# craftsangjae/instance-segmentation-road-project

Measured on AMD Instinct MI355X. Metric: images/sec at 1024x1024 (MaskLab inference hot path, full forward), higher is better.
Workload: dtype f32; 1 GPU; resnext50_full_b8_1024; per_gpu_batch=8, global_batch=8, height=1024, width=1024, parallelism=dp1, hipgraph=False, inputs=resident in HBM, weights=random init (cls logits x8 so NMS / mask head run at full load)

## Files before the change

### include/masklab_hip.h

```cpp
#ifndef MASKLAB_HIP_H
#define MASKLAB_HIP_H

#include <stdint.h>

#ifdef __cplusplus
extern "C" {
#endif

#define ML_OK 0
#define ML_E_BADARG (-1)
#define ML_E_LAUNCH (-2)
#define ML_E_NOGPU  (-3)

enum { ML_ACT_NONE = 0, ML_ACT_RELU = 1, ML_ACT_RELU6 = 2, ML_ACT_SIGMOID = 3 };
enum { ML_MATH_F32 = 0, ML_MATH_F16 = 1, ML_MATH_F16S = 2, ML_MATH_F32X3 = 3 };

#define ML_ABI_VERSION 7
int ml_version(void);
const char *ml_last_error(void);
int ml_device_check(void);

typedef struct ml_conv2d_desc {
    const float *in;
    const float *wgt;
// ... 25 lines not shown
} ml_conv2d_desc;

int ml_conv2d_f32(const ml_conv2d_desc *d, void *stream);

#define ML_CONV_MAX_PROBLEMS 12
int64_t ml_conv2d_workspace_bytes(void);
int ml_conv2d_multi_f32(const ml_conv2d_desc *descs, int32_t n, void *workspace, int64_t workspace_bytes,
                        void *stream);
int ml_conv2d_ntile(int32_t cout, int32_t tile);
int ml_conv2d_launch_ntile(const ml_conv2d_desc *descs, int32_t n, int32_t has_workspace);
int ml_conv2d_launch_mtile(const ml_conv2d_desc *descs, int32_t n, int32_t has_workspace);
int ml_conv2d_uses_pipe(const ml_conv2d_desc *d);
int ml_conv2d_launch_splits(const ml_conv2d_desc *descs, int32_t n, int64_t workspace_bytes, int32_t *splits);
int ml_conv2d_wino_eligible(const ml_conv2d_desc *d);
int ml_conv2d_wino_narrow(const ml_conv2d_desc *d);
int64_t ml_conv2d_gn_min_launch_tiles(void);

int ml_gconv3x3_f32(const float *in, const float *wgt, const float *bias, float *out,
                    int32_t B, int32_t H, int32_t W, int32_t C, int32_t c, int32_t Ho, int32_t Wo,
                    int32_t stride, int32_t pad_t, int32_t pad_l, int32_t act, void *stream);

int ml_gconv3x3_f16(const void *in, const float *wgt, const float *bias, void *out,
                    int32_t B, int32_t H, int32_t W, int32_t C, int32_t c, int32_t Ho, int32_t Wo,
                    int32_t stride, int32_t pad_t, int32_t pad_l, int32_t act, void *stream);

int ml_gconv3x3_launch_plan(int32_t B, int32_t H, int32_t W, int32_t C, int32_t c, int32_t stride, int32_t Ho, int32_t Wo,
                            int32_t is_half, int32_t plan[6]);

int ml_maxpool3x3s2_f16(const void *in, void *out, int32_t B, int32_t H, int32_t W, int32_t C,
                        int32_t Ho, int32_t Wo, int32_t pad_t, int32_t pad_l, void *stream);
// ... 397 lines not shown
```

### instance-segmentation-road-project_amd/csrc/conv_mfma.hip

```cpp
#include "gfx_mem.h"

namespace {

constexpr int LDS_LD = 32;
constexpr int LDS_LD_H = 40;

constexpr int MAXP = ML_CONV_MAX_PROBLEMS;

struct FastDiv { unsigned mul; int shift; };

static FastDiv make_fastdiv(unsigned d) {
    FastDiv f;
    if (d <= 1) { f.mul = 0; f.shift = -1; return f; }
    int s = 0;
    while ((1ull << s) < d) ++s;
    const unsigned long long num = 1ull << (31 + s);
    f.mul = (unsigned)((num + d - 1) / d);
    f.shift = s - 1;
    return f;
}

__device__ __forceinline__ int fast_div(int n, const FastDiv f) {
    return f.shift < 0 ? n : (int)(__umulhi((unsigned)n, f.mul) >> f.shift);
}
// ... 992 lines not shown
                       "vector epilogue (out / bias 16-byte aligned, out_cstride and out_coff multiples of 4)");
        p.start[i] = (int)start;
        start += (MB + 7) / 8 * 8 * (d.n_pad / p.BN) * splits;
        ML_REQUIRE(start < (1ll << 31), "conv2d: grid too large");
    }
    p.start[p.n] = (int)start;
    return ML_OK;
}

}

int ml_conv1x1_pipe_try(const ml_conv2d_desc &d, hipStream_t s, int *eligible);
int ml_conv1x1_pipe_eligible(const ml_conv2d_desc &d);
int ml_conv1x1_h256_try(const ml_conv2d_desc &d, hipStream_t s, int *took);
int ml_conv1x1_h256_eligible(const ml_conv2d_desc &d);
int ml_conv2d_wino_launch(const ml_conv2d_desc *descs, int n, hipStream_t s);

static bool h256_preferred(const ml_conv2d_desc &d) {
    return d.tile == 5 || (d.tile == 0 && (d.span >= 512 || (d.span >= 256 && d.cout >= 512)));
}

extern "C" int ml_conv2d_ntile(int32_t cout, int32_t tile) {
    const int t = pick_tile(cout, tile);
    return t == 1 ? 128 : (t == 2 ? 64 : 32);
}

extern "C" int64_t ml_conv2d_workspace_bytes(void) { return 512ll << 20; }

static int split_by_image_groups(const ml_conv2d_desc *descs, int n, ConvPlan &p) {
    p.n = 0;
    for (int i = 0; i < n; ++i) {
// ... 128 lines not shown
    }
    ML_REQUIRE(p.kernel < N_GENERIC_KERNELS, "conv2d: no kernel instantiation for math %d, %d x %d tiles", math, p.BM, p.BN);
    return check ? plan_splits(p, ws_bytes) : ML_OK;
}

extern "C" int ml_conv2d_multi_f32(const ml_conv2d_desc *descs, int32_t n, void *workspace, int64_t workspace_bytes,
                                   void *stream) {
    ML_REQUIRE(descs != nullptr && n >= 1 && n <= MAXP, "conv2d: need 1..%d problems", MAXP);
    for (int i = 0; i < n; ++i) {
        ML_REQUIRE(descs[i].in && descs[i].wgt && descs[i].out, "conv2d: null tensor pointer");
        ML_REQUIRE(ml_aligned16(descs[i].in) && ml_aligned16(descs[i].wgt), "conv2d: in/wgt must be 16-byte aligned");
    }
    ConvPlan p;
    if (int rc = plan_launch(descs, n, workspace ? workspace_bytes : 0, p)) return rc;
    hipStream_t s = reinterpret_cast<hipStream_t>(stream);
    if (p.family == CONV_WINO) return ml_conv2d_wino_launch(descs, n, s);
    if (p.family == CONV_H256 || p.family == CONV_PIPE) {
        int took = 0;
        if (int rc = (p.family == CONV_H256 ? ml_conv1x1_h256_try : ml_conv1x1_pipe_try)(descs[0], s, &took)) return rc;
        ML_REQUIRE(took, "conv2d: the persistent 1x1 kernel did not take a problem it was planned for");
        return ML_OK;
    }
    if (workspace) ML_REQUIRE((((uintptr_t)workspace) & 255) == 0, "conv2d: workspace must be 256-byte aligned");
    return kGenericKernels[p.kernel].launch(p, workspace, s);
}


extern "C" int ml_conv2d_uses_pipe(const ml_conv2d_desc *d) {
    ConvPlan p;
    return plan_launch(d, 1, 0, p, false) != ML_OK ? 0 : (p.family == CONV_H256 ? 2 : p.family == CONV_PIPE);
}

extern "C" int ml_conv2d_launch_ntile(const ml_conv2d_desc *descs, int32_t n, int32_t has_workspace) {
    ConvPlan p;
    return plan_launch(descs, n, has_workspace ? ml_conv2d_workspace_bytes() : 0, p, false) == ML_OK && p.family == CONV_GENERIC ? p.BN : 0;
}

extern "C" int ml_conv2d_launch_mtile(const ml_conv2d_desc *descs, int32_t n, int32_t has_workspace) {
    ConvPlan p;
// ... 24 lines not shown
```

### instance-segmentation-road-project_amd/csrc/conv_wino.hip

```cpp
#include "gfx_mem.h"

namespace {

constexpr int WMAXP = ML_CONV_MAX_PROBLEMS;
constexpr int WT = 64;
constexpr int WN = 64;
constexpr int WK = 8;
constexpr int WCHUNK = WK * 32 * 16;
constexpr int WSTEP = 4 * 32 * 16;
constexpr int NSLOT_P = 3;
constexpr int SLOT_P = WT * 16 * 8;
constexpr int NSLOT_W = 4;
constexpr int SLOT_W = 2 * WSTEP;
constexpr int RING_W = NSLOT_P * SLOT_P;
constexpr int LDS_BYTES = (RING_W + NSLOT_W * SLOT_W) * 4;
static_assert(LDS_BYTES == 160 * 1024, "the two rings fill the CU's LDS");
#ifndef WINO_EXP
#define WINO_EXP 0
#endif
constexpr unsigned OOB = 0x80000000u;
constexpr long long SPAN_MAX = 0x7fffff00ll;

struct WProblem {
    ml_conv2d_desc d;
    int TH, TW, T;
    int MB, NB, nchunks;
};

struct WArgs {
    int n;
    int start[WMAXP + 1];
    WProblem p[WMAXP];
};

typedef f32x4 f32x4d __attribute__((aligned(4)));

__device__ __forceinline__ void out_store(float *base, float *ptr, float val) {
#if (WINO_EXP & 8) && defined(__HIP_DEVICE_COMPILE__)
    const __amdgpu_buffer_rsrc_t none = rsrc_bytes(base, 0);
    __builtin_amdgcn_raw_buffer_store_b32(__builtin_bit_cast(unsigned, val), none, (int)((ptr - base) * 4), 0, 0);
#else
// ... 27 lines not shown
            default: v[i * 4 + 3] = t[i * 4 + 1] - t[i * 4 + 3]; break;
        }
    }
}

__global__ void __launch_bounds__(512, 1) conv_wino_kernel(const WArgs args) {
    extern __shared__ __align__(16) float lds[];

    int pi = 0;
    while (pi + 1 < args.n && (int)blockIdx.x >= args.start[pi + 1]) ++pi;
    const WProblem &P = args.p[pi];
    const ml_conv2d_desc &p = P.d;
    const int b = (int)blockIdx.x - args.start[pi];
    const int g = b / (8 * P.NB), rr = b - g * 8 * P.NB;
    const int nt2 = rr >> 3;
    const int mt = g * 8 + (rr & 7);
    if (mt >= P.MB) return;
    if (p.live) {
        const int lv = max(1, *p.live), tpi0 = P.TH * P.TW;
        const int b0 = mt * WT / tpi0, b1 = min(mt * WT + WT, P.T) - 1;
        bool any = false;
        for (int bi = b0; bi <= b1 / tpi0 && !any; ++bi) any = bi % p.live_period < lv;
        if (!any) return;
    }

    const int tid = threadIdx.x, lane = tid & 63;
    const int wave = __builtin_amdgcn_readfirstlane(tid >> 6);
    const int tg = wave & 3, h = wave >> 2;
    const int r = lane & 15, kq = lane >> 4;
    const int tpi = P.TH * P.TW;

    const int gt0 = mt * WT;
    long long base_pix;
    {
        const int bi = gt0 / tpi, rem = gt0 - bi * tpi, ty = rem / P.TW;
        base_pix = ((long long)bi * p.H + max(2 * ty - 1, 0)) * p.W;
    }
    const size_t cstride = (size_t)p.in_cstride;
    const float *pin = p.in + p.in_coff + (size_t)base_pix * cstride;
    int voff_p[4];
    {
        const int rt = (lane >> 1) & 15;
        const int quad = (lane & 1) ^ ((rt >> 2) & 1);
        const int gt = gt0 + (wave >> 1) * 16 + rt;
        int bi = 0, ty = 0, tx = 0;
        if (gt < P.T) {
            bi = gt / tpi;
            const int rem = gt - bi * tpi;
            ty = rem / P.TW;
            tx = rem - ty * P.TW;
        }
#pragma unroll
        for (int i = 0; i < 4; ++i) {
            const int px = 8 * (wave & 1) + 2 * i + (lane >> 5);
            const int y = 2 * ty - 1 + (px >> 2), x = 2 * tx - 1 + (px & 3);
            voff_p[i] = (int)OOB;
            if (gt < P.T && y >= 0 && y < p.H && x >= 0 && x < p.W)
                voff_p[i] = (int)((((long long)bi * p.H + y) * p.W + x - base_pix) * (long long)cstride * 4) + quad * 16;
        }
    }
    const int voff_w = ((wave & 3) * 512 + r * 16 + kq * 4) * 4;
    const float *wsrc = p.wgt + (size_t)(2 * nt2 + (wave >> 2)) * P.nchunks * WCHUNK;
    float *dst_p = lds + (wave >> 1) * 2048 + (wave & 1) * 1024;
    float *dst_w = lds + RING_W + (wave >> 2) * WSTEP + (wave & 3) * 512;
    const int nch = P.nchunks, nsteps = 2 * P.nchunks;
    const bool dead = (2 * nt2 + h) * 32 >= p.cout;

    auto rsrc_p = [&](int j) __attribute__((always_inline)) {
        const bool real = j < nch && !(WINO_EXP & 1);
        return rsrc_bytes(pin + j * 8, real ? (int)OOB : 0);
    };
    auto rsrc_w = [&](int s) __attribute__((always_inline)) {
        const bool real = s < nsteps && !dead && !(WINO_EXP & 2);
        return rsrc_bytes(wsrc + (size_t)s * WSTEP, real ? WSTEP * 4 : 0);
    };

    f32x4 acc[2][16];
#pragma unroll
    for (int t = 0; t < 2; ++t)
#pragma unroll
        for (int q = 0; q < 16; ++q) acc[t][q] = f32x4{0.f, 0.f, 0.f, 0.f};

    const float *pa_lane0 = lds + tg * 2048 + r * 8 + 4 * ((r >> 2) & 1) + kq;
    const float *pa_lane1 = lds + tg * 2048 + r * 8 + 4 * (((r >> 2) & 1) ^ 1) + kq;
    const float *pb_lane = lds + RING_W + h * WSTEP + kq * 512 + r * 4;
    struct Ops {
        float d[16], t[16], v[16];
        f32x4 b[2][4];
    };
    auto read_ops = [&](const float *pa, const float *pb, Ops &o) __attribute__((always_inline)) {
#pragma unroll
        for (int t = 0; t < 2; ++t)
#pragma unroll
            for (int pq = 0; pq < 4; ++pq) o.b[t][pq] = *reinterpret_cast<const f32x4 *>(pb + t * 256 + pq * 64);
#pragma unroll
        for (int px = 0; px < 16; ++px) o.d[px] = pa[px * 128];
// ... 18 lines not shown
#if WINO_EXP != 4
            if (m % 6 == 5 && m / 6 < ndma) {
                __builtin_amdgcn_sched_barrier(0);
                dma(m / 6);
                __builtin_amdgcn_sched_barrier(0);
            }
#endif
            if (m >= 16) {
                bt_d_b_op(2 * (m - 16), nxt.d, nxt.t, nxt.v);
                bt_d_b_op(2 * (m - 16) + 1, nxt.d, nxt.t, nxt.v);
                __builtin_amdgcn_sched_barrier(0);
            }
        }
    };

    {
        const __amdgpu_buffer_rsrc_t rp0 = rsrc_p(0), rp1 = rsrc_p(1), rw0 = rsrc_w(0), rw1 = rsrc_w(1), rw2 = rsrc_w(2);
#pragma unroll
        for (int i = 0; i < 4; ++i) lds_dma16(rp0, (char *)(dst_p + i * 256), voff_p[i], 0);
        lds_dma16(rw0, (char *)dst_w, voff_w, 0);
        lds_dma16(rw0, (char *)(dst_w + 256), voff_w + 1024, 0);
#pragma unroll
        for (int i = 0; i < 4; ++i) lds_dma16(rp1, (char *)(dst_p + SLOT_P + i * 256), voff_p[i], 0);
        lds_dma16(rw1, (char *)(dst_w + SLOT_W), voff_w, 0);
        lds_dma16(rw1, (char *)(dst_w + SLOT_W + 256), voff_w + 1024, 0);
        lds_dma16(rw2, (char *)(dst_w + 2 * SLOT_W), voff_w, 0);
        lds_dma16(rw2, (char *)(dst_w + 2 * SLOT_W + 256), voff_w + 1024, 0);
    }
    wait_vmcnt<8>();
    __builtin_amdgcn_s_barrier();

    if (dead) {
        int ps2 = 2 * SLOT_P;
        for (int j = 0; j < nch; ++j) {
            const int w0 = (2 * j) & 3;
            const int wa = ((w0 ^ 2) + 1) * SLOT_W, wb = w0 * SLOT_W;
            asm volatile("s_waitcnt vmcnt(0) lgkmcnt(0)" ::: "memory");
            __builtin_amdgcn_s_barrier();
            const __amdgpu_buffer_rsrc_t rp = rsrc_p(j + 2), rwa = rsrc_w(2 * j + 3), rwb = rsrc_w(2 * j + 4);
#pragma unroll
            for (int q = 0; q < 8; ++q) {
                if (q < 4) lds_dma16(rp, (char *)(dst_p + ps2 + q * 256), voff_p[q], 0);
                else if (q < 6) lds_dma16(rwa, (char *)(dst_w + wa + (q - 4) * 256), voff_w + (q - 4) * 1024, 0);
                else lds_dma16(rwb, (char *)(dst_w + wb + (q - 6) * 256), voff_w + (q - 6) * 1024, 0);
                __builtin_amdgcn_s_sleep(3);
            }
            ps2 = ps2 == 2 * SLOT_P ? 0 : ps2 + SLOT_P;
        }
        wait_vmcnt<0>();
        return;
    }

    Ops oa, ob;
    read_ops(pa_lane0, pb_lane, oa);
#pragma unroll
    for (int k = 0; k < 32; ++k) bt_d_b_op(k, oa.d, oa.t, oa.v);

    int ps0 = 0, ps1 = SLOT_P, ps2 = 2 * SLOT_P;
    for (int j = 0; j < nch; ++j) {
        const int w0 = (2 * j) & 3;
        const int wa = ((w0 ^ 2) + 1) * SLOT_W, wb = w0 * SLOT_W;
        asm volatile("s_waitcnt vmcnt(0) lgkmcnt(0)" ::: "memory");
        __builtin_amdgcn_s_barrier();
        const __amdgpu_buffer_rsrc_t rp = rsrc_p(j + 2), rwa = rsrc_w(2 * j + 3), rwb = rsrc_w(2 * j + 4);
        auto dma = [&](int q) __attribute__((always_inline)) {
            if (q < 4) lds_dma16(rp, (char *)(dst_p + ps2 + q * 256), voff_p[q], 0);
            else if (q < 6) lds_dma16(rwa, (char *)(dst_w + wa + (q - 4) * 256), voff_w + (q - 4) * 1024, 0);
            else lds_dma16(rwb, (char *)(dst_w + wb + (q - 6) * 256), voff_w + (q - 6) * 1024, 0);
        };
        step(oa, ob, pa_lane1 + ps0, pb_lane + (w0 + 1) * SLOT_W, 5, dma);
        step(ob, oa, pa_lane0 + ps1, pb_lane + (w0 ^ 2) * SLOT_W, 3, [&](int q) __attribute__((always_inline)) { dma(q + 5); });
        const int ps = ps0;
        ps0 = ps1;
        ps1 = ps2;
        ps2 = ps;
    }
    wait_vmcnt<0>();

    const int nt = 2 * nt2 + h;
    const bool gn = p.gn_partials != nullptr && !(WINO_EXP & 16);
    double gs[2] = {0.0, 0.0}, gq[2] = {0.0, 0.0};
    long long f0 = 0;
    if (gn) {
        const int bi = gt0 / tpi, rem = gt0 - bi * tpi, ty = rem / P.TW, tx = rem - ty * P.TW;
        f0 = ((long long)(bi * p.Ho + 2 * ty) * p.Wo + 2 * tx) >> 7;
    }
    const float lo = 0.f, hi = (p.act == ML_ACT_RELU6) ? 6.f : 3.402823466e38f;
    const bool clampv = p.act == ML_ACT_RELU || p.act == ML_ACT_RELU6;
    const int gt = gt0 + tg * 16 + r;
    if (gt < P.T) {
        const int bi = gt / tpi, rem = gt - bi * tpi;
        const int ty = rem / P.TW, tx = rem - ty * P.TW;
        const int oy = 2 * ty, ox = 2 * tx;
        const bool y1 = oy + 1 < p.Ho, x1 = ox + 1 < p.Wo;
        const size_t img = p.out_bstride ? (size_t)bi * (size_t)p.out_bstride : (size_t)bi * p.Ho * p.Wo * p.out_cstride;
        const size_t pix0 = (size_t)oy * p.Wo + ox;
        const long long m_flat0 = (long long)(bi * p.Ho + oy) * p.Wo + ox;
#pragma unroll
        for (int t = 0; t < 2; ++t) {
            const int n = nt * 32 + 16 * t + 4 * kq;
            if (n >= p.cout) continue;
            const bool quad = n + 4 <= p.cout;
            f32x4 u[8];
#pragma unroll
            for (int j = 0; j < 4; ++j) {
                u[j] = acc[t][0 * 4 + j] + acc[t][1 * 4 + j] + acc[t][2 * 4 + j];
                u[4 + j] = acc[t][1 * 4 + j] - acc[t][2 * 4 + j] - acc[t][3 * 4 + j];
            }
            f32x4 bv = {0.f, 0.f, 0.f, 0.f};
            if (p.bias) {
                if (quad) bv = *reinterpret_cast<const f32x4d *>(p.bias + n);
                else
#pragma unroll
                    for (int c = 0; c < 3; ++c)
                        if (n + c < p.cout) bv[c] = p.bias[n + c];
            }
            float *o = p.out + img + p.out_coff + n;
#pragma unroll
            for (int a = 0; a < 2; ++a)
#pragma unroll
                for (int c2 = 0; c2 < 2; ++c2) {
                    if ((a && !y1) || (c2 && !x1)) continue;
                    f32x4 val = (c2 ? u[4 * a + 1] - u[4 * a + 2] - u[4 * a + 3] : u[4 * a + 0] + u[4 * a + 1] + u[4 * a + 2]) + bv;
#pragma unroll
                    for (int c = 0; c < 4; ++c) {
                        if (clampv) val[c] = __builtin_amdgcn_fmed3f(val[c], lo, hi);
                        else if (p.act != ML_ACT_NONE) val[c] = ml_apply_act(val[c], p.act);
                    }
                    float *op = o + (pix0 + (size_t)a * p.Wo + c2) * p.out_cstride;
                    if (quad) out_store(p.out, op, val);
                    else
#pragma unroll
                        for (int c = 0; c < 3; ++c)
                            if (n + c < p.cout) out_store(p.out, op + c, val[c]);
                    if (gn) {
                        const int f = ((m_flat0 + (long long)a * p.Wo + c2) >> 7) != f0;
#pragma unroll
                        for (int c = 0; c < 4; ++c) {
                            gs[f] += (double)val[c];
                            gq[f] += (double)val[c] * (double)val[c];
                        }
                    }
                }
        }
    }
    if (gn) {
        double *lds_gn = reinterpret_cast<double *>(lds);
        __syncthreads();
#pragma unroll
        for (int o = 32; o > 0; o >>= 1) {
#pragma unroll
            for (int f = 0; f < 2; ++f) {
                gs[f] += __shfl_down(gs[f], o, 64);
                gq[f] += __shfl_down(gq[f], o, 64);
            }
        }
        if (lane == 0) {
            lds_gn[wave * 4 + 0] = gs[0]; lds_gn[wave * 4 + 1] = gq[0];
            lds_gn[wave * 4 + 2] = gs[1]; lds_gn[wave * 4 + 3] = gq[1];
        }
        __syncthreads();
        if (tid < 4) {
            const int hh = tid >> 1, ff = tid & 1;
            const int gt1 = gt0 + WT - 1;
            const int bi = gt1 / tpi, rem = gt1 - bi * tpi, ty = rem / P.TW, tx = rem - ty * P.TW;
            const long long f1 = ((long long)(bi * p.Ho + 2 * ty + 1) * p.Wo + 2 * tx + 1) >> 7;
            const long long ft = ff ? f1 : f0;
            const int slot = 2 * nt2 + hh;
            double s = 0.0, q = 0.0;
            for (int w = 0; w < 4; ++w) { s += lds_gn[(hh * 4 + w) * 4 + 2 * ff]; q += lds_gn[(hh * 4 + w) * 4 + 2 * ff + 1]; }
            p.gn_partials[2 * (ft * 4 + slot)] = s;
            p.gn_partials[2 * (ft * 4 + slot) + 1] = q;
        }
    }
}

}

extern "C" int ml_conv2d_wino_eligible(const ml_conv2d_desc *d) {
    if (!d) return 0;
    return d->math == ML_MATH_F32 && d->KH == 3 && d->KW == 3 && d->stride == 1 && d->dil == 1 && d->pad_t == 1 &&
           d->pad_l == 1 && d->Ho == d->H && d->Wo == d->W && d->cpp_shift == 30 && d->group_cin_step == 0 &&
           !d->shuffle2x2 && !d->residual && !d->out_f16 && d->span % 32 == 0 && d->span_pad == d->span &&
           d->cout <= 128 && d->n_pad == 128;
}

extern "C" int ml_conv2d_wino_narrow(const ml_conv2d_desc *d) {
    if (!d || d->live || d->gn_partials) return 0;
    if (d->n_pad != 32 && d->n_pad != 64 && d->n_pad != 96) return 0;
    if (d->cout < 1 || d->cout > d->n_pad || d->cout == 32 || d->cout == 64) return 0;
    ml_conv2d_desc w = *d;
    w.n_pad = 128;
    return ml_conv2d_wino_eligible(&w);
}

int ml_conv2d_wino_gn_ok(const ml_conv2d_desc &d) {
    if (d.Ho % 2 || d.Wo % 2 || d.cout != 128 || d.out_bstride || d.act == ML_ACT_SIGMOID) return 0;
    const long long TH = d.Ho / 2, TW = d.Wo / 2;
    return (64 % TW == 0 || TW % 64 == 0) && (TH * TW) % 64 == 0;
}

int ml_conv2d_wino_launch(const ml_conv2d_desc *descs, int n, hipStream_t s) {
    ML_REQUIRE(n >= 1 && n <= WMAXP, "conv2d (winograd): need 1..%d problems", WMAXP);
    WArgs args;
    args.n = n;
    long long start = 0;
    for (int i = 0; i < n; ++i) {
        const ml_conv2d_desc &d = descs[i];
        ML_REQUIRE(ml_conv2d_wino_eligible(&d),
                   "conv2d: tile = 6 (Winograd F(2x2,3x3)) needs ML_MATH_F32, a 3x3 stride-1 undilated 'same' conv, no "
                   "groups / shuffle / residual / half output, span %% 32 == 0 and n_pad == 128");
        ML_REQUIRE(((d.in_cstride | d.in_coff) & 3) == 0 && ml_aligned16(d.in) && ml_aligned16(d.wgt),
                   "conv2d (winograd): 16-byte aligned input channels and weights");
        if (d.gn_partials)
            ML_REQUIRE(ml_conv2d_wino_gn_ok(d) && !d.live, "conv2d (winograd): gn_partials needs even Ho / Wo, Wo / 2 dividing or a "
                                                "multiple of 64, (Ho / 2) (Wo / 2) %% 64 == 0, cout = 128, dense output");
        WProblem &P = args.p[i];
        P.d = d;
        P.TH = (d.Ho + 1) / 2;
        P.TW = (d.Wo + 1) / 2;
        const long long T = (long long)d.B * P.TH * P.TW;
        ML_REQUIRE(T < (1ll << 30), "conv2d (winograd): too many tiles");
        P.T = (int)T;
        P.MB = (int)((T + WT - 1) / WT);
        P.NB = (d.cout + WN - 1) / WN;
        P.nchunks = d.span_pad / WK;
        const long long span = (2ll * (WT / P.TW + 2) + 2) * d.W * d.in_cstride * 4;
        ML_REQUIRE(span <= SPAN_MAX, "conv2d (winograd): a block's input rows exceed 2 GiB (W x in_cstride too large)");
        args.start[i] = (int)start;
        start += (long long)(P.MB + 7) / 8 * 8 * P.NB;
        ML_REQUIRE(start < (1ll << 31), "conv2d (winograd): grid too large");
    }
    args.start[n] = (int)start;
    long long tiles128 = 0;
    bool any_gn = false;
    for (int i = 0; i < n; ++i) {
        tiles128 += ((long long)descs[i].B * descs[i].Ho * descs[i].Wo + 127) / 128 * (descs[i].n_pad / 128);
        any_gn = any_gn || descs[i].gn_partials != nullptr;
    }
    ML_REQUIRE(!any_gn || tiles128 >= ml_conv2d_gn_min_launch_tiles(),
               "conv2d (winograd): gn_partials needs a launch of ml_conv2d_gn_min_launch_tiles() tiles of 128 x 128");
    static std::atomic<unsigned long long> lds_ok{0};
    if (int rc = ml_ensure_dynamic_lds(reinterpret_cast<const void *>(conv_wino_kernel), LDS_BYTES, lds_ok, "conv2d (winograd)"))
        return rc;
    hipLaunchKernelGGL(conv_wino_kernel, dim3((unsigned)start), dim3(512), LDS_BYTES, s, args);
    ML_CHECK_LAUNCH("conv2d (winograd)");
    return ML_OK;
}
// ... 1 lines not shown
```

### instance-segmentation-road-project_amd/masklab_hip/_lib.py

```python
import ctypes as C
import os

_HERE = os.path.dirname(os.path.abspath(__file__))
LIB_PATH = os.path.join(_HERE, "libmasklab_hip.so")

ABI_VERSION = 7
ACT_NONE, ACT_RELU, ACT_RELU6, ACT_SIGMOID = 0, 1, 2, 3
ACT_BY_NAME = {None: ACT_NONE, "linear": ACT_NONE, "relu": ACT_RELU, "relu6": ACT_RELU6,
               "sigmoid": ACT_SIGMOID}


class ConvDesc(C.Structure):
    _fields_ = [
        ("in_", C.c_void_p), ("wgt", C.c_void_p), ("bias", C.c_void_p),
        ("residual", C.c_void_p), ("out", C.c_void_p),
        ("B", C.c_int32), ("H", C.c_int32), ("W", C.c_int32),
        ("in_cstride", C.c_int32), ("in_coff", C.c_int32),
        ("span", C.c_int32), ("span_pad", C.c_int32), ("cpp_shift", C.c_int32),
        ("Ho", C.c_int32), ("Wo", C.c_int32),
        ("KH", C.c_int32), ("KW", C.c_int32), ("stride", C.c_int32), ("dil", C.c_int32),
        ("pad_t", C.c_int32), ("pad_l", C.c_int32),
        ("cout", C.c_int32), ("n_pad", C.c_int32),
        ("out_cstride", C.c_int32), ("out_coff", C.c_int32),
        ("res_cstride", C.c_int32), ("res_coff", C.c_int32),
# ... 74 lines not shown
DECONV_OUT_MAX_PROBLEMS = 4
_i32, _i64, _f32, _f64, _vp = C.c_int32, C.c_int64, C.c_float, C.c_double, C.c_void_p

SIGNATURES = {
    "ml_version": (C.c_int, []),
    "ml_last_error": (C.c_char_p, []),
    "ml_device_check": (C.c_int, []),
    "ml_conv2d_f32": (C.c_int, [C.POINTER(ConvDesc), _vp]),
    "ml_conv2d_ntile": (C.c_int, [_i32, _i32]),
    "ml_conv2d_uses_pipe": (C.c_int, [C.POINTER(ConvDesc)]),
    "ml_conv2d_launch_ntile": (C.c_int, [C.POINTER(ConvDesc), _i32, _i32]),
    "ml_conv2d_launch_mtile": (C.c_int, [C.POINTER(ConvDesc), _i32, _i32]),
    "ml_conv2d_launch_splits": (C.c_int, [C.POINTER(ConvDesc), _i32, _i64, C.POINTER(C.c_int32)]),
    "ml_conv2d_wino_eligible": (C.c_int, [C.POINTER(ConvDesc)]),
    "ml_conv2d_wino_narrow": (C.c_int, [C.POINTER(ConvDesc)]),
    "ml_conv2d_gn_min_launch_tiles": (_i64, []),
    "ml_conv2d_workspace_bytes": (_i64, []),
    "ml_conv2d_multi_f32": (C.c_int, [C.POINTER(ConvDesc), _i32, _vp, _i64, _vp]),
    "ml_deconv2x2_out1x1_f32": (C.c_int, [C.POINTER(DeconvOutProblem), _i32, _i32, _i32, _i32, _i32, _i32, _i32, _vp]),
    "ml_gconv3x3_f32": (C.c_int, [_vp, _vp, _vp, _vp] + [_i32] * 11 + [_vp]),
    "ml_gconv3x3_f16": (C.c_int, [_vp, _vp, _vp, _vp] + [_i32] * 11 + [_vp]),
    "ml_gconv3x3_launch_plan": (C.c_int, [_i32] * 9 + [C.POINTER(C.c_int32)]),
    "ml_maxpool3x3s2_f16": (C.c_int, [_vp, _vp] + [_i32] * 8 + [_vp]),
    "ml_stem7x7s2_pool_f16": (C.c_int, [_vp, _vp, _vp, _vp] + [_i32] * 5 + [_vp]),
    "ml_stem7x7s2_pool_f32": (C.c_int, [_vp, _vp, _vp, _vp] + [_i32] * 5 + [_vp]),
    "ml_stem7x7s2_pool_x3": (C.c_int, [_vp, _vp, _vp, _vp] + [_i32] * 5 + [_vp]),
    "ml_subsample2_f16": (C.c_int, [_vp, _vp] + [_i32] * 4 + [_vp]),
    "ml_cast_f16_to_f32": (C.c_int, [_vp, _vp, _i64, _vp]),
    "ml_cast_f32_to_f16": (C.c_int, [_vp, _vp, _i64, _vp]),
    "ml_resize_bilinear_ac_f16": (C.c_int, [_vp, _vp, _vp] + [_i32] * 12 + [_vp]),
# ... 147 lines not shown
```

### instance-segmentation-road-project_amd/masklab_hip/ops.py

```python
import ctypes as C
import threading

import numpy as np
import torch

from . import _lib
from .packing import PackedConv, pack_winograd, resolve_padding

import weakref

_ws_cache = {}
_ws_retired = []
_graph_owners = weakref.WeakSet()


def graph_owner_registered(model):
    _graph_owners.add(model)


def graph_owner_released(model):
    _graph_owners.discard(model)
    if not len(_graph_owners):
        _ws_retired.clear()

PROFILE = None
LAUNCH_LOG = None


class _Prof:
    def __init__(self, kernel, flops, nbytes, shape=""):
        self.on = PROFILE is not None
        if self.on:
            self.rec = {"kernel": kernel, "flops": float(flops), "bytes": float(nbytes), "shape": shape,
                        "start": torch.cuda.Event(enable_timing=True), "end": torch.cuda.Event(enable_timing=True)}

    def __enter__(self):
        if self.on:
            self.rec["start"].record()
        return self

    def __exit__(self, *exc):
# ... 217 lines not shown
    if wino:
        flops = sum(_wino_flops(descs[i]) for i in range(n))
    ws = workspace(int(lib.ml_conv2d_workspace_bytes()), x.device, "conv")
    if LAUNCH_LOG is not None:
        sp = (C.c_int32 * n)()
        _lib.check(lib.ml_conv2d_launch_splits(descs, n, ws.numel(), sp), "ml_conv2d_launch_splits")
        LAUNCH_LOG.append((" | ".join(shapes) if multi else label, tuple(int(v) for v in sp)))
    name = None
    if PROFILE is not None:
        name = "conv_wino_f32" if wino else _conv_kernel_name(descs, n, dc.p, x.dtype == torch.float16)
    with _Prof(name, flops, nbytes, label) as prof:
        if prof.on and name == "conv1x1_h256_h":
            d = descs[0]
            M, N, K = d.B * d.Ho * d.Wo, d.cout, d.span
            prof.rec["staged_bytes"] = float(-(-M // 256) * (N // 256) * 2 * 256 * K * 2)
        _lib.check(lib.ml_conv2d_multi_f32(descs, n, _ptr(ws), ws.numel(), _stream()), "ml_conv2d_multi_f32")


def _wino_select(descs, n, problems):
    if CONV_MATH != "f32":
        return False
    lib = _lib.load()
    for i, (x, dc) in enumerate(problems):
        if x.dtype != torch.float32 or dc.p.tile != 0:
            return False
        if not (lib.ml_conv2d_wino_eligible(C.byref(descs[i])) or lib.ml_conv2d_wino_narrow(C.byref(descs[i]))):
            return False
    for i, (x, dc) in enumerate(problems):
        descs[i].tile, descs[i].n_pad = 6, 128
        descs[i].wgt = dc.wgt_wino.data_ptr()
    return True
# ... 2047 lines not shown
```

Measured before the change: 436.2 images/sec.

## Make Winograd conv blocks persistent over multiple M panels with cross-panel prefetch

Restructures the Winograd F(2x2,3x3) kernel so one block can loop over several consecutive M panels. The next panel's input and weight DMA is staged into LDS during the current panel's epilogue, and the bias load moves to buffer loads. This is meant to hide prologue latency and cut block launch overhead. The default panel count from wino_class_panels is 1, so the multi-panel path only runs when WINO_PANELS is set, and the default path still carries the restructured loop and extra barriers.

Result: no change. 436.5 images/sec, median of 2 (+0.0%).

```diff
diff --git a/include/masklab_hip.h b/include/masklab_hip.h
--- a/include/masklab_hip.h
+++ b/include/masklab_hip.h
@@ -63,6 +63,8 @@
 int ml_conv2d_launch_splits(const ml_conv2d_desc *descs, int32_t n, int64_t workspace_bytes, int32_t *splits);
 int ml_conv2d_wino_eligible(const ml_conv2d_desc *d);
 int ml_conv2d_wino_narrow(const ml_conv2d_desc *d);
+int ml_conv2d_wino_launch_plan(const ml_conv2d_desc *descs, int32_t n, int32_t *plan);
+int ml_conv2d_multi_wino_panels_f32(const ml_conv2d_desc *descs, int32_t n, const int32_t *panels, void *stream);
 int64_t ml_conv2d_gn_min_launch_tiles(void);
 
 int ml_gconv3x3_f32(const float *in, const float *wgt, const float *bias, float *out,
diff --git a/instance-segmentation-road-project_amd/csrc/conv_mfma.hip b/instance-segmentation-road-project_amd/csrc/conv_mfma.hip
--- a/instance-segmentation-road-project_amd/csrc/conv_mfma.hip
+++ b/instance-segmentation-road-project_amd/csrc/conv_mfma.hip
@@ -1030,7 +1030,7 @@
 int ml_conv1x1_pipe_eligible(const ml_conv2d_desc &d);
 int ml_conv1x1_h256_try(const ml_conv2d_desc &d, hipStream_t s, int *took);
 int ml_conv1x1_h256_eligible(const ml_conv2d_desc &d);
-int ml_conv2d_wino_launch(const ml_conv2d_desc *descs, int n, hipStream_t s);
+int ml_conv2d_wino_launch(const ml_conv2d_desc *descs, int n, const int32_t *panels, hipStream_t s);
 
 static bool h256_preferred(const ml_conv2d_desc &d) {
     return d.tile == 5 || (d.tile == 0 && (d.span >= 512 || (d.span >= 256 && d.cout >= 512)));
@@ -1189,7 +1189,7 @@
     ConvPlan p;
     if (int rc = plan_launch(descs, n, workspace ? workspace_bytes : 0, p)) return rc;
     hipStream_t s = reinterpret_cast<hipStream_t>(stream);
-    if (p.family == CONV_WINO) return ml_conv2d_wino_launch(descs, n, s);
+    if (p.family == CONV_WINO) return ml_conv2d_wino_launch(descs, n, nullptr, s);
     if (p.family == CONV_H256 || p.family == CONV_PIPE) {
         int took = 0;
         if (int rc = (p.family == CONV_H256 ? ml_conv1x1_h256_try : ml_conv1x1_pipe_try)(descs[0], s, &took)) return rc;
@@ -1198,6 +1198,18 @@
     }
     if (workspace) ML_REQUIRE((((uintptr_t)workspace) & 255) == 0, "conv2d: workspace must be 256-byte aligned");
     return kGenericKernels[p.kernel].launch(p, workspace, s);
+}
+
+extern "C" int ml_conv2d_multi_wino_panels_f32(const ml_conv2d_desc *descs, int32_t n, const int32_t *panels, void *stream) {
+    ML_REQUIRE(descs != nullptr && panels != nullptr && n >= 1 && n <= MAXP, "conv2d: need 1..%d problems", MAXP);
+    for (int i = 0; i < n; ++i) {
+        ML_REQUIRE(descs[i].in && descs[i].wgt && descs[i].out, "conv2d: null tensor pointer");
+        ML_REQUIRE(ml_aligned16(descs[i].in) && ml_aligned16(descs[i].wgt), "conv2d: in/wgt must be 16-byte aligned");
+    }
+    ConvPlan p;
+    if (int rc = plan_launch(descs, n, 0, p)) return rc;
+    ML_REQUIRE(p.family == CONV_WINO, "conv2d: panels per block are a choice of the Winograd kernel (tile = 6) only");
+    return ml_conv2d_wino_launch(descs, n, panels, reinterpret_cast<hipStream_t>(stream));
 }
 
 
diff --git a/instance-segmentation-road-project_amd/csrc/conv_wino.hip b/instance-segmentation-road-project_amd/csrc/conv_wino.hip
--- a/instance-segmentation-road-project_amd/csrc/conv_wino.hip
+++ b/instance-segmentation-road-project_amd/csrc/conv_wino.hip
@@ -25,6 +25,7 @@
     ml_conv2d_desc d;
     int TH, TW, T;
     int MB, NB, nchunks;
+    int kp, GB;
 };
 
 struct WArgs {
@@ -82,32 +83,39 @@
     const int b = (int)blockIdx.x - args.start[pi];
     const int g = b / (8 * P.NB), rr = b - g * 8 * P.NB;
     const int nt2 = rr >> 3;
-    const int mt = g * 8 + (rr & 7);
-    if (mt >= P.MB) return;
-    if (p.live) {
-        const int lv = max(1, *p.live), tpi0 = P.TH * P.TW;
-        const int b0 = mt * WT / tpi0, b1 = min(mt * WT + WT, P.T) - 1;
-        bool any = false;
-        for (int bi = b0; bi <= b1 / tpi0 && !any; ++bi) any = bi % p.live_period < lv;
-        if (!any) return;
-    }
+    const int mt_first = (g * 8 + (rr & 7)) * P.kp;
+    const int mt_end = min(mt_first + P.kp, P.MB);
+    const int tpi = P.TH * P.TW;
+    const int lv = p.live ? max(1, *p.live) : 0;
+    auto next_panel = [&](int mt) __attribute__((always_inline)) {
+        for (; mt < mt_end; ++mt) {
+            if (!p.live) break;
+            const int b0 = mt * WT / tpi, b1 = min(mt * WT + WT, P.T) - 1;
+            bool any = false;
+            for (int bi = b0; bi <= b1 / tpi && !any; ++bi) any = bi % p.live_period < lv;
+            if (any) break;
+        }
+        return mt;
+    };
+    int mt = next_panel(mt_first);
+    if (mt >= mt_end) return;
 
     const int tid = threadIdx.x, lane = tid & 63;
     const int wave = __builtin_amdgcn_readfirstlane(tid >> 6);
     const int tg = wave & 3, h = wave >> 2;
     const int r = lane & 15, kq = lane >> 4;
-    const int tpi = P.TH * P.TW;
-
-    const int gt0 = mt * WT;
-    long long base_pix;
-    {
-        const int bi = gt0 / tpi, rem = gt0 - bi * tpi, ty = rem / P.TW;
-        base_pix = ((long long)bi * p.H + max(2 * ty - 1, 0)) * p.W;
-    }
+
     const size_t cstride = (size_t)p.in_cstride;
-    const float *pin = p.in + p.in_coff + (size_t)base_pix * cstride;
+    const float *pin;
     int voff_p[4];
-    {
+    auto panel_geometry = [&](int mtp) __attribute__((always_inline)) {
+        const int gt0 = mtp * WT;
+        long long base_pix;
+        {
+            const int bi = gt0 / tpi, rem = gt0 - bi * tpi, ty = rem / P.TW;
+            base_pix = ((long long)bi * p.H + max(2 * ty - 1, 0)) * p.W;
+        }
+        pin = p.in + p.in_coff + (size_t)base_pix * cstride;
         const int rt = (lane >> 1) & 15;
         const int quad = (lane & 1) ^ ((rt >> 2) & 1);
         const int gt = gt0 + (wave >> 1) * 16 + rt;
@@ -126,7 +134,8 @@
             if (gt < P.T && y >= 0 && y < p.H && x >= 0 && x < p.W)
                 voff_p[i] = (int)((((long long)bi * p.H + y) * p.W + x - base_pix) * (long long)cstride * 4) + quad * 16;
         }
-    }
+    };
+    panel_geometry(mt);
     const int voff_w = ((wave & 3) * 512 + r * 16 + kq * 4) * 4;
     const float *wsrc = p.wgt + (size_t)(2 * nt2 + (wave >> 2)) * P.nchunks * WCHUNK;
     float *dst_p = lds + (wave >> 1) * 2048 + (wave & 1) * 1024;
@@ -144,10 +153,6 @@
     };
 
     f32x4 acc[2][16];
-#pragma unroll
-    for (int t = 0; t < 2; ++t)
-#pragma unroll
-        for (int q = 0; q < 16; ++q) acc[t][q] = f32x4{0.f, 0.f, 0.f, 0.f};
 
     const float *pa_lane0 = lds + tg * 2048 + r * 8 + 4 * ((r >> 2) & 1) + kq;
     const float *pa_lane1 = lds + tg * 2048 + r * 8 + 4 * (((r >> 2) & 1) ^ 1) + kq;
@@ -196,8 +201,10 @@
         }
     };
 
-    {
-        const __amdgpu_buffer_rsrc_t rp0 = rsrc_p(0), rp1 = rsrc_p(1), rw0 = rsrc_w(0), rw1 = rsrc_w(1), rw2 = rsrc_w(2);
+    auto prologue = [&]() __attribute__((always_inline)) {
+        const bool none = (WINO_EXP & 32) != 0;
+        const __amdgpu_buffer_rsrc_t rp0 = rsrc_p(none ? nch : 0), rp1 = rsrc_p(none ? nch : 1);
+        const __amdgpu_buffer_rsrc_t rw0 = rsrc_w(none ? nsteps : 0), rw1 = rsrc_w(none ? nsteps : 1), rw2 = rsrc_w(none ? nsteps : 2);
 #pragma unroll
         for (int i = 0; i < 4; ++i) lds_dma16(rp0, (char *)(dst_p + i * 256), voff_p[i], 0);
         lds_dma16(rw0, (char *)dst_w, voff_w, 0);
@@ -208,152 +215,192 @@
         lds_dma16(rw1, (char *)(dst_w + SLOT_W + 256), voff_w + 1024, 0);
         lds_dma16(rw2, (char *)(dst_w + 2 * SLOT_W), voff_w, 0);
         lds_dma16(rw2, (char *)(dst_w + 2 * SLOT_W + 256), voff_w + 1024, 0);
-    }
+    };
+    auto stage_next = [&](int nx) __attribute__((always_inline)) {
+        if (nx < mt_end) {
+            asm volatile("s_waitcnt vmcnt(0) lgkmcnt(0)" ::: "memory");
+            __builtin_amdgcn_s_barrier();
+            panel_geometry(nx);
+            prologue();
+        }
+    };
+    auto enter_staged = [&]() __attribute__((always_inline)) {
+        asm volatile("s_waitcnt vmcnt(0) lgkmcnt(0)" ::: "memory");
+        __builtin_amdgcn_s_barrier();
+    };
+    auto clear_acc = [&]() __attribute__((always_inline)) {
+#pragma unroll
+        for (int t = 0; t < 2; ++t)
+#pragma unroll
+            for (int q = 0; q < 16; ++q) {
+                acc[t][q] = f32x4{0.f, 0.f, 0.f, 0.f};
+                asm volatile("" : "+v"(acc[t][q]));
+            }
+    };
+    prologue();
+    clear_acc();
     wait_vmcnt<8>();
     __builtin_amdgcn_s_barrier();
 
     if (dead) {
-        int ps2 = 2 * SLOT_P;
+        for (;;) {
+            int ps2 = 2 * SLOT_P;
+            for (int j = 0; j < nch; ++j) {
+                const int w0 = (2 * j) & 3;
+                const int wa = ((w0 ^ 2) + 1) * SLOT_W, wb = w0 * SLOT_W;
+                asm volatile("s_waitcnt vmcnt(0) lgkmcnt(0)" ::: "memory");
+                __builtin_amdgcn_s_barrier();
+                const __amdgpu_buffer_rsrc_t rp = rsrc_p(j + 2), rwa = rsrc_w(2 * j + 3), rwb = rsrc_w(2 * j + 4);
+#pragma unroll
+                for (int q = 0; q < 8; ++q) {
+                    if (q < 4) lds_dma16(rp, (char *)(dst_p + ps2 + q * 256), voff_p[q], 0);
+                    else if (q < 6) lds_dma16(rwa, (char *)(dst_w + wa + (q - 4) * 256), voff_w + (q - 4) * 1024, 0);
+                    else lds_dma16(rwb, (char *)(dst_w + wb + (q - 6) * 256), voff_w + (q - 6) * 1024, 0);
+                    __builtin_amdgcn_s_sleep(3);
+                }
+                ps2 = ps2 == 2 * SLOT_P ? 0 : ps2 + SLOT_P;
+            }
+            wait_vmcnt<0>();
+            mt = next_panel(mt + 1);
+            stage_next(mt);
+            if (mt >= mt_end) return;
+            enter_staged();
+        }
+    }
+
+    for (;;) {
+        Ops oa, ob;
+        read_ops(pa_lane0, pb_lane, oa);
+#pragma unroll
+        for (int k = 0; k < 32; ++k) bt_d_b_op(k, oa.d, oa.t, oa.v);
+
+        int ps0 = 0, ps1 = SLOT_P, ps2 = 2 * SLOT_P;
         for (int j = 0; j < nch; ++j) {
             const int w0 = (2 * j) & 3;
             const int wa = ((w0 ^ 2) + 1) * SLOT_W, wb = w0 * SLOT_W;
             asm volatile("s_waitcnt vmcnt(0) lgkmcnt(0)" ::: "memory");
             __builtin_amdgcn_s_barrier();
             const __amdgpu_buffer_rsrc_t rp = rsrc_p(j + 2), rwa = rsrc_w(2 * j + 3), rwb = rsrc_w(2 * j + 4);
-#pragma unroll
-            for (int q = 0; q < 8; ++q) {
+            auto dma = [&](int q) __attribute__((always_inline)) {
                 if (q < 4) lds_dma16(rp, (char *)(dst_p + ps2 + q * 256), voff_p[q], 0);
                 else if (q < 6) lds_dma16(rwa, (char *)(dst_w + wa + (q - 4) * 256), voff_w + (q - 4) * 1024, 0);
                 else lds_dma16(rwb, (char *)(dst_w + wb + (q - 6) * 256), voff_w + (q - 6) * 1024, 0);
-                __builtin_amdgcn_s_sleep(3);
-            }
-            ps2 = ps2 == 2 * SLOT_P ? 0 : ps2 + SLOT_P;
+            };
+            step(oa, ob, pa_lane1 + ps0, pb_lane + (w0 + 1) * SLOT_W, 5, dma);
+            step(ob, oa, pa_lane0 + ps1, pb_lane + (w0 ^ 2) * SLOT_W, 3, [&](int q) __attribute__((always_inline)) { dma(q + 5); });
+            const int ps = ps0;
+            ps0 = ps1;
+            ps1 = ps2;
+            ps2 = ps;
         }
         wait_vmcnt<0>();
-        return;
-    }
-
-    Ops oa, ob;
-    read_ops(pa_lane0, pb_lane, oa);
-#pragma unroll
-    for (int k = 0; k < 32; ++k) bt_d_b_op(k, oa.d, oa.t, oa.v);
-
-    int ps0 = 0, ps1 = SLOT_P, ps2 = 2 * SLOT_P;
-    for (int j = 0; j < nch; ++j) {
-        const int w0 = (2 * j) & 3;
-        const int wa = ((w0 ^ 2) + 1) * SLOT_W, wb = w0 * SLOT_W;
-        asm volatile("s_waitcnt vmcnt(0) lgkmcnt(0)" ::: "memory");
-        __builtin_amdgcn_s_barrier();
-        const __amdgpu_buffer_rsrc_t rp = rsrc_p(j + 2), rwa = rsrc_w(2 * j + 3), rwb = rsrc_w(2 * j + 4);
-        auto dma = [&](int q) __attribute__((always_inline)) {
-            if (q < 4) lds_dma16(rp, (char *)(dst_p + ps2 + q * 256), voff_p[q], 0);
-            else if (q < 6) lds_dma16(rwa, (char *)(dst_w + wa + (q - 4) * 256), voff_w + (q - 4) * 1024, 0);
-            else lds_dma16(rwb, (char *)(dst_w + wb + (q - 6) * 256), voff_w + (q - 6) * 1024, 0);
-        };
-        step(oa, ob, pa_lane1 + ps0, pb_lane + (w0 + 1) * SLOT_W, 5, dma);
-        step(ob, oa, pa_lane0 + ps1, pb_lane + (w0 ^ 2) * SLOT_W, 3, [&](int q) __attribute__((always_inline)) { dma(q + 5); });
-        const int ps = ps0;
-        ps0 = ps1;
-        ps1 = ps2;
-        ps2 = ps;
-    }
-    wait_vmcnt<0>();
-
-    const int nt = 2 * nt2 + h;
-    const bool gn = p.gn_partials != nullptr && !(WINO_EXP & 16);
-    double gs[2] = {0.0, 0.0}, gq[2] = {0.0, 0.0};
-    long long f0 = 0;
-    if (gn) {
-        const int bi = gt0 / tpi, rem = gt0 - bi * tpi, ty = rem / P.TW, tx = rem - ty * P.TW;
-        f0 = ((long long)(bi * p.Ho + 2 * ty) * p.Wo + 2 * tx) >> 7;
-    }
-    const float lo = 0.f, hi = (p.act == ML_ACT_RELU6) ? 6.f : 3.402823466e38f;
-    const bool clampv = p.act == ML_ACT_RELU || p.act == ML_ACT_RELU6;
-    const int gt = gt0 + tg * 16 + r;
-    if (gt < P.T) {
-        const int bi = gt / tpi, rem = gt - bi * tpi;
-        const int ty = rem / P.TW, tx = rem - ty * P.TW;
-        const int oy = 2 * ty, ox = 2 * tx;
-        const bool y1 = oy + 1 < p.Ho, x1 = ox + 1 < p.Wo;
-        const size_t img = p.out_bstride ? (size_t)bi * (size_t)p.out_bstride : (size_t)bi * p.Ho * p.Wo * p.out_cstride;
-        const size_t pix0 = (size_t)oy * p.Wo + ox;
-        const long long m_flat0 = (long long)(bi * p.Ho + oy) * p.Wo + ox;
-#pragma unroll
-        for (int t = 0; t < 2; ++t) {
-            const int n = nt * 32 + 16 * t + 4 * kq;
-            if (n >= p.cout) continue;
-            const bool quad = n + 4 <= p.cout;
-            f32x4 u[8];
-#pragma unroll
-            for (int j = 0; j < 4; ++j) {
-                u[j] = acc[t][0 * 4 + j] + acc[t][1 * 4 + j] + acc[t][2 * 4 + j];
-                u[4 + j] = acc[t][1 * 4 + j] - acc[t][2 * 4 + j] - acc[t][3 * 4 + j];
-            }
-            f32x4 bv = {0.f, 0.f, 0.f, 0.f};
-            if (p.bias) {
-                if (quad) bv = *reinterpret_cast<const f32x4d *>(p.bias + n);
-                else
-#pragma unroll
-                    for (int c = 0; c < 3; ++c)
-                        if (n + c < p.cout) bv[c] = p.bias[n + c];
-            }
-            float *o = p.out + img + p.out_coff + n;
-#pragma unroll
-            for (int a = 0; a < 2; ++a)
-#pragma unroll
-                for (int c2 = 0; c2 < 2; ++c2) {
-                    if ((a && !y1) || (c2 && !x1)) continue;
-                    f32x4 val = (c2 ? u[4 * a + 1] - u[4 * a + 2] - u[4 * a + 3] : u[4 * a + 0] + u[4 * a + 1] + u[4 * a + 2]) + bv;
-#pragma unroll
-                    for (int c = 0; c < 4; ++c) {
-                        if (clampv) val[c] = __builtin_amdgcn_fmed3f(val[c], lo, hi);
-                        else if (p.act != ML_ACT_NONE) val[c] = ml_apply_act(val[c], p.act);
-                    }
-                    float *op = o + (pix0 + (size_t)a * p.Wo + c2) * p.out_cstride;
-                    if (quad) out_store(p.out, op, val);
-                    else
-#pragma unroll
-                        for (int c = 0; c < 3; ++c)
-                            if (n + c < p.cout) out_store(p.out, op + c, val[c]);
-                    if (gn) {
-                        const int f = ((m_flat0 + (long long)a * p.Wo + c2) >> 7) != f0;
+
+        const int nt = 2 * nt2 + h;
+        f32x4 bias_v[2];
+        {
+            const i32x4 rb = rsrc_words(p.bias, p.bias ? p.cout * 4 : 0);
+#pragma unroll
+            for (int t = 0; t < 2; ++t) bias_v[t] = buf_load16_asm(rb, (nt * 32 + 16 * t + 4 * kq) * 4);
+        }
+        const int gt0 = mt * WT;
+        mt = next_panel(mt + 1);
+        const bool more = mt < mt_end;
+        if (more) wait_loaded<0>(bias_v[0], bias_v[1]);
+        stage_next(mt);
+        const bool gn = p.gn_partials != nullptr && !(WINO_EXP & 16);
+        double gs[2] = {0.0, 0.0}, gq[2] = {0.0, 0.0};
+        long long f0 = 0;
+        if (gn) {
+            const int bi = gt0 / tpi, rem = gt0 - bi * tpi, ty = rem / P.TW, tx = rem - ty * P.TW;
+            f0 = ((long long)(bi * p.Ho + 2 * ty) * p.Wo + 2 * tx) >> 7;
+        }
+        const float lo = 0.f, hi = (p.act == ML_ACT_RELU6) ? 6.f : 3.402823466e38f;
+        const bool clampv = p.act == ML_ACT_RELU || p.act == ML_ACT_RELU6;
+        const int gt = gt0 + tg * 16 + r;
+        if (gt < P.T) {
+            const int bi = gt / tpi, rem = gt - bi * tpi;
+            const int ty = rem / P.TW, tx = rem - ty * P.TW;
+            const int oy = 2 * ty, ox = 2 * tx;
+            const bool y1 = oy + 1 < p.Ho, x1 = ox + 1 < p.Wo;
+            const size_t img = p.out_bstride ? (size_t)bi * (size_t)p.out_bstride : (size_t)bi * p.Ho * p.Wo * p.out_cstride;
+            const size_t pix0 = (size_t)oy * p.Wo + ox;
+            const long long m_flat0 = (long long)(bi * p.Ho + oy) * p.Wo + ox;
+            if (!more) wait_loaded<0>(bias_v[0], bias_v[1]);
+#pragma unroll
+            for (int t = 0; t < 2; ++t) {
+                const int n = nt * 32 + 16 * t + 4 * kq;
+                if (n >= p.cout) continue;
+                const bool quad = n + 4 <= p.cout;
+                f32x4 u[8];
+#pragma unroll
+                for (int j = 0; j < 4; ++j) {
+                    u[j] = acc[t][0 * 4 + j] + acc[t][1 * 4 + j] + acc[t][2 * 4 + j];
+                    u[4 + j] = acc[t][1 * 4 + j] - acc[t][2 * 4 + j] - acc[t][3 * 4 + j];
+                }
+                const f32x4 bv = bias_v[t];
+                float *o = p.out + img + p.out_coff + n;
+#pragma unroll
+                for (int a = 0; a < 2; ++a)
+#pragma unroll
+                    for (int c2 = 0; c2 < 2; ++c2) {
+                        if ((a && !y1) || (c2 && !x1)) continue;
+                        f32x4 val = (c2 ? u[4 * a + 1] - u[4 * a + 2] - u[4 * a + 3] : u[4 * a + 0] + u[4 * a + 1] + u[4 * a + 2]) + bv;
 #pragma unroll
                         for (int c = 0; c < 4; ++c) {
-                            gs[f] += (double)val[c];
-                            gq[f] += (double)val[c] * (double)val[c];
+                            if (clampv) val[c] = __builtin_amdgcn_fmed3f(val[c], lo, hi);
+                            else if (p.act != ML_ACT_NONE) val[c] = ml_apply_act(val[c], p.act);
+                        }
+                        float *op = o + (pix0 + (size_t)a * p.Wo + c2) * p.out_cstride;
+                        if (quad) out_store(p.out, op, val);
+                        else
+#pragma unroll
+                            for (int c = 0; c < 3; ++c)
+                                if (n + c < p.cout) out_store(p.out, op + c, val[c]);
+                        if (gn) {
+                            const int f = ((m_flat0 + (long long)a * p.Wo + c2) >> 7) != f0;
+#pragma unroll
+                            for (int c = 0; c < 4; ++c) {
+                                gs[f] += (double)val[c];
+                                gq[f] += (double)val[c] * (double)val[c];
+                            }
                         }
                     }
+            }
+        }
+        if (gn) {
+            double *lds_gn = reinterpret_cast<double *>(lds + RING_W + 3 * SLOT_W);
+            asm volatile("s_waitcnt lgkmcnt(0)" ::: "memory");
+            __builtin_amdgcn_s_barrier();
+#pragma unroll
+            for (int o = 32; o > 0; o >>= 1) {
+#pragma unroll
+                for (int f = 0; f < 2; ++f) {
+                    gs[f] += __shfl_down(gs[f], o, 64);
+                    gq[f] += __shfl_down(gq[f], o, 64);
                 }
-        }
-    }
-    if (gn) {
-        double *lds_gn = reinterpret_cast<double *>(lds);
-        __syncthreads();
-#pragma unroll
-        for (int o = 32; o > 0; o >>= 1) {
-#pragma unroll
-            for (int f = 0; f < 2; ++f) {
-                gs[f] += __shfl_down(gs[f], o, 64);
-                gq[f] += __shfl_down(gq[f], o, 64);
-            }
-        }
-        if (lane == 0) {
-            lds_gn[wave * 4 + 0] = gs[0]; lds_gn[wave * 4 + 1] = gq[0];
-            lds_gn[wave * 4 + 2] = gs[1]; lds_gn[wave * 4 + 3] = gq[1];
-        }
-        __syncthreads();
-        if (tid < 4) {
-            const int hh = tid >> 1, ff = tid & 1;
-            const int gt1 = gt0 + WT - 1;
-            const int bi = gt1 / tpi, rem = gt1 - bi * tpi, ty = rem / P.TW, tx = rem - ty * P.TW;
-            const long long f1 = ((long long)(bi * p.Ho + 2 * ty + 1) * p.Wo + 2 * tx + 1) >> 7;
-            const long long ft = ff ? f1 : f0;
-            const int slot = 2 * nt2 + hh;
-            double s = 0.0, q = 0.0;
-            for (int w = 0; w < 4; ++w) { s += lds_gn[(hh * 4 + w) * 4 + 2 * ff]; q += lds_gn[(hh * 4 + w) * 4 + 2 * ff + 1]; }
-            p.gn_partials[2 * (ft * 4 + slot)] = s;
-            p.gn_partials[2 * (ft * 4 + slot) + 1] = q;
-        }
+            }
+            if (lane == 0) {
+                lds_gn[wave * 4 + 0] = gs[0]; lds_gn[wave * 4 + 1] = gq[0];
+                lds_gn[wave * 4 + 2] = gs[1]; lds_gn[wave * 4 + 3] = gq[1];
+            }
+            asm volatile("s_waitcnt lgkmcnt(0)" ::: "memory");
+            __builtin_amdgcn_s_barrier();
+            if (tid < 4) {
+                const int hh = tid >> 1, ff = tid & 1;
+                const int gt1 = gt0 + WT - 1;
+                const int bi = gt1 / tpi, rem = gt1 - bi * tpi, ty = rem / P.TW, tx = rem - ty * P.TW;
+                const long long f1 = ((long long)(bi * p.Ho + 2 * ty + 1) * p.Wo + 2 * tx + 1) >> 7;
+                const long long ft = ff ? f1 : f0;
+                const int slot = 2 * nt2 + hh;
+                double s = 0.0, q = 0.0;
+                for (int w = 0; w < 4; ++w) { s += lds_gn[(hh * 4 + w) * 4 + 2 * ff]; q += lds_gn[(hh * 4 + w) * 4 + 2 * ff + 1]; }
+                p.gn_partials[2 * (ft * 4 + slot)] = s;
+                p.gn_partials[2 * (ft * 4 + slot) + 1] = q;
+            }
+        }
+        if (mt >= mt_end) return;
+        clear_acc();
+        enter_staged();
     }
 }
 
@@ -382,9 +429,13 @@
     return (64 % TW == 0 || TW % 64 == 0) && (TH * TW) % 64 == 0;
 }
 
-int ml_conv2d_wino_launch(const ml_conv2d_desc *descs, int n, hipStream_t s) {
-    ML_REQUIRE(n >= 1 && n <= WMAXP, "conv2d (winograd): need 1..%d problems", WMAXP);
-    WArgs args;
+static int wino_class_panels(const ml_conv2d_desc &d) {
+    (void)d;
+    return 1;
+}
+
+static int wino_plan(const ml_conv2d_desc *descs, int n, const int32_t *force, WArgs &args) {
+    ML_REQUIRE(descs != nullptr && n >= 1 && n <= WMAXP, "conv2d (winograd): need 1..%d problems", WMAXP);
     args.n = n;
     long long start = 0;
     for (int i = 0; i < n; ++i) {
@@ -392,8 +443,7 @@
         ML_REQUIRE(ml_conv2d_wino_eligible(&d),
                    "conv2d: tile = 6 (Winograd F(2x2,3x3)) needs ML_MATH_F32, a 3x3 stride-1 undilated 'same' conv, no "
                    "groups / shuffle / residual / half output, span %% 32 == 0 and n_pad == 128");
-        ML_REQUIRE(((d.in_cstride | d.in_coff) & 3) == 0 && ml_aligned16(d.in) && ml_aligned16(d.wgt),
-                   "conv2d (winograd): 16-byte aligned input channels and weights");
+        ML_REQUIRE(((d.in_cstride | d.in_coff) & 3) == 0, "conv2d (winograd): 16-byte aligned input channels and weights");
         if (d.gn_partials)
             ML_REQUIRE(ml_conv2d_wino_gn_ok(d) && !d.live, "conv2d (winograd): gn_partials needs even Ho / Wo, Wo / 2 dividing or a "
                                                 "multiple of 64, (Ho / 2) (Wo / 2) %% 64 == 0, cout = 128, dense output");
@@ -402,18 +452,46 @@
         P.TH = (d.Ho + 1) / 2;
         P.TW = (d.Wo + 1) / 2;
         const long long T = (long long)d.B * P.TH * P.TW;
-        ML_REQUIRE(T < (1ll << 30), "conv2d (winograd): too many tiles");
+        ML_REQUIRE(T >= 1 && T < (1ll << 30), "conv2d (winograd): too many tiles");
         P.T = (int)T;
         P.MB = (int)((T + WT - 1) / WT);
         P.NB = (d.cout + WN - 1) / WN;
         P.nchunks = d.span_pad / WK;
+        if (force) {
+            ML_REQUIRE(force[i] >= 1 && force[i] <= 64, "conv2d (winograd): 1..64 panels per block");
+            P.kp = force[i];
+        } else {
+            P.kp = wino_class_panels(d);
+            if (P.MB < P.kp) P.kp = 1;
+        }
+        P.GB = (P.MB + P.kp - 1) / P.kp;
         const long long span = (2ll * (WT / P.TW + 2) + 2) * d.W * d.in_cstride * 4;
         ML_REQUIRE(span <= SPAN_MAX, "conv2d (winograd): a block's input rows exceed 2 GiB (W x in_cstride too large)");
         args.start[i] = (int)start;
-        start += (long long)(P.MB + 7) / 8 * 8 * P.NB;
+        start += (long long)(P.GB + 7) / 8 * 8 * P.NB;
         ML_REQUIRE(start < (1ll << 31), "conv2d (winograd): grid too large");
     }
     args.start[n] = (int)start;
+    return ML_OK;
+}
+
+extern "C" int ml_conv2d_wino_launch_plan(const ml_conv2d_desc *descs, int32_t n, int32_t *plan) {
+    ML_REQUIRE(plan != nullptr, "conv2d (winograd): null plan");
+    WArgs args;
+    if (int rc = wino_plan(descs, n, nullptr, args)) return rc;
+    for (int i = 0; i < n; ++i) {
+        plan[2 * i] = args.p[i].kp;
+        plan[2 * i + 1] = args.start[i + 1] - args.start[i];
+    }
+    return ML_OK;
+}
+
+int ml_conv2d_wino_launch(const ml_conv2d_desc *descs, int n, const int32_t *panels, hipStream_t s) {
+    WArgs args;
+    if (int rc = wino_plan(descs, n, panels, args)) return rc;
+    for (int i = 0; i < n; ++i)
+        ML_REQUIRE(ml_aligned16(descs[i].in) && ml_aligned16(descs[i].wgt), "conv2d (winograd): 16-byte aligned input channels and weights");
+    const long long start = args.start[n];
     long long tiles128 = 0;
     bool any_gn = false;
     for (int i = 0; i < n; ++i) {
diff --git a/instance-segmentation-road-project_amd/masklab_hip/_lib.py b/instance-segmentation-road-project_amd/masklab_hip/_lib.py
--- a/instance-segmentation-road-project_amd/masklab_hip/_lib.py
+++ b/instance-segmentation-road-project_amd/masklab_hip/_lib.py
@@ -112,6 +112,8 @@
     "ml_conv2d_launch_splits": (C.c_int, [C.POINTER(ConvDesc), _i32, _i64, C.POINTER(C.c_int32)]),
     "ml_conv2d_wino_eligible": (C.c_int, [C.POINTER(ConvDesc)]),
     "ml_conv2d_wino_narrow": (C.c_int, [C.POINTER(ConvDesc)]),
+    "ml_conv2d_wino_launch_plan": (C.c_int, [C.POINTER(ConvDesc), _i32, C.POINTER(C.c_int32)]),
+    "ml_conv2d_multi_wino_panels_f32": (C.c_int, [C.POINTER(ConvDesc), _i32, C.POINTER(C.c_int32), _vp]),
     "ml_conv2d_gn_min_launch_tiles": (_i64, []),
     "ml_conv2d_workspace_bytes": (_i64, []),
     "ml_conv2d_multi_f32": (C.c_int, [C.POINTER(ConvDesc), _i32, _vp, _i64, _vp]),
diff --git a/instance-segmentation-road-project_amd/masklab_hip/ops.py b/instance-segmentation-road-project_amd/masklab_hip/ops.py
--- a/instance-segmentation-road-project_amd/masklab_hip/ops.py
+++ b/instance-segmentation-road-project_amd/masklab_hip/ops.py
@@ -25,6 +25,7 @@
 
 PROFILE = None
 LAUNCH_LOG = None
+WINO_PANELS = None
 
 
 class _Prof:
@@ -272,7 +273,14 @@
             d = descs[0]
             M, N, K = d.B * d.Ho * d.Wo, d.cout, d.span
             prof.rec["staged_bytes"] = float(-(-M // 256) * (N // 256) * 2 * 256 * K * 2)
-        _lib.check(lib.ml_conv2d_multi_f32(descs, n, _ptr(ws), ws.numel(), _stream()), "ml_conv2d_multi_f32")
+        if wino and WINO_PANELS is not None:
+            ks = list(WINO_PANELS) if isinstance(WINO_PANELS, (list, tuple)) else [int(WINO_PANELS)] * n
+            if len(ks) != n:
+                raise ValueError(f"WINO_PANELS: {len(ks)} values for a launch of {n} problems")
+            _lib.check(lib.ml_conv2d_multi_wino_panels_f32(descs, n, (C.c_int32 * n)(*ks), _stream()),
+                       "ml_conv2d_multi_wino_panels_f32")
+        else:
+            _lib.check(lib.ml_conv2d_multi_f32(descs, n, _ptr(ws), ws.numel(), _stream()), "ml_conv2d_multi_f32")
 
 
 def _wino_select(descs, n, problems):
```
